# mpieva/mapping-iterative-assembler

Hardware: AMD Instinct MI355X
Metric: reads aligned/sec per iteration (16.5kb mito ref, 100bp reads) (higher is better)
Workload: dtype int32; 1 GPU; configs[1]: 1000000 synthetic 100 bp reads per GPU vs mt311 (16619 bp, circular), matrix flat; step = reiterate_assembly + pop_smp + cull + consensus; pass-1 coordinates = true positions; reads_per_gpu=1000000, total_reads=1000000, consensus_len=16619, bytes_per_read=182

## Files before the change

mapping-iterative-assembler_amd/csrc/mia_consensus_kernels.h:

```cpp
#pragma once
#include <hip/hip_runtime.h>
#include <stdint.h>

#include "mia_kernels.h"
#include "mia_layout.h"

namespace mia {

struct TallyBuf {
  int32_t* tally;
  int32_t Lp;
  int32_t* gaps;
  uint64_t* events;
  int32_t* n_events;
  int32_t cap_events;
  uint32_t* flags;
};

struct RecGeom {
  int start_w, end, split, ncols_f, ncols_b;
};
MIA_HD inline RecGeom rec_geom(int as, int ae, int L) {
  RecGeom g;
  g.start_w = as;
  g.end = ae > L ? ae - L : ae;
  g.split = as > g.end;
  g.ncols_f = g.split ? (L - as) : (g.end - as + 1);
  g.ncols_b = g.split ? g.end + 1 : 0;
  return g;
}

__global__ void k_scan_blocks(ReadSet rs, int32_t L, int64_t* partial) {
  __shared__ int32_t sh[256];
  const int64_t base = ((int64_t)blockIdx.x * 256 + threadIdx.x) * 16;
  int32_t s = 0;
  for (int k = 0; k < 16; k++) {
    int64_t i = base + k;
    if (i < rs.n && rs.sk[i]) s += rec_geom(rs.as[i], rs.ae[i], L).split ? 2 : 1;
  }
  sh[threadIdx.x] = s;
  __syncthreads();
  for (int o = 128; o > 0; o >>= 1) {
    if ((int)threadIdx.x < o) sh[threadIdx.x] += sh[threadIdx.x + o];
    __syncthreads();
  }
  if (threadIdx.x == 0) partial[blockIdx.x] = sh[0];
}
__global__ __launch_bounds__(256) void k_scan_partials(int64_t* partial, int nb, int64_t base, int64_t* total, const int32_t* abort_if = nullptr) {
  if (abort_if && *abort_if != 0) return;
  __shared__ int64_t s_run[256];
  const int t = threadIdx.x, per = (nb + 255) / 256, b0 = t * per, b1 = b0 + per < nb ? b0 + per : nb;
  int64_t mine = 0;
  for (int b = b0; b < b1; b++) mine += partial[b];
  const int lane = t & 63, w = t >> 6;
  int64_t inc = mine;
#pragma unroll
  for (int o = 1; o < 64; o <<= 1) { const int64_t u = (int64_t)__shfl_up((long long)inc, o); if (lane >= o) inc += u; }
  if (lane == 63) s_run[w] = inc;
// ... 782 lines not shown
    if (e < last) {
      const int32_t v = order[e];
      rd[q] = packed ? (v & 0xFFFFFF) : v;
      key[q] = packed ? (int)((uint32_t)v >> 24) : (int)okey[e];
      rank[q] = atomicAdd(&h[key[q]], 1);
    }
  }
  const int mine = pre[t];
  for (int o = 1; o < SORT2_KEYS; o <<= 1) {
    __syncthreads();
    const int v = t >= o ? pre[t - o] : 0;
    __syncthreads();
    pre[t] += v;
  }
  __syncthreads();
  pre[t] -= mine;
  base[t] = h[t] ? atomicAdd(&cursor2[(int64_t)b * SORT2_KEYS + t], h[t]) : 0;
  __syncthreads();
  const int ob = off[b];
#pragma unroll
  for (int q = 0; q < PER; q++)
    if (rd[q] >= 0) order2[ob + pre[key[q]] + base[key[q]] + rank[q]] = rd[q];
}

#ifdef MIA_HIP_ALT_PATHS
__device__ unsigned long long g_tally_kinds[8];
#define TALLY_KIND(k) do { if (dbg & 65536u) atomicAdd(&g_tally_kinds[k], 1ull); } while (0)
__device__ unsigned long long g_tally_clk[8];
#define TALLY_CLK(k) do { if ((dbg & 131072u) && threadIdx.x == 0) { const unsigned long long now_ = __builtin_amdgcn_s_memtime(); atomicAdd(&g_tally_clk[k], now_ - clk_); clk_ = now_; } } while (0)
#define TALLY_CLK_DECL unsigned long long clk_ = (dbg & 131072u) ? __builtin_amdgcn_s_memtime() : 0ull
#define TALLY_ABL(bit) ((dbg & (bit)) != 0u)
#else
#define TALLY_ABL(bit) false
#define TALLY_KIND(k) do { } while (0)
#define TALLY_CLK(k) do { } while (0)
#define TALLY_CLK_DECL do { } while (0)
#endif
__device__ __forceinline__ uint32_t wave_transpose32(uint32_t x, int lane) {
#pragma unroll
  for (int j = 16; j >= 1; j >>= 1) {
    const uint32_t m = j == 16 ? 0x0000FFFFu : (j == 8 ? 0x00FF00FFu : (j == 4 ? 0x0F0F0F0Fu : (j == 2 ? 0x33333333u : 0x55555555u)));
    const uint32_t y = (uint32_t)__shfl_xor((int)x, j);
    x = (lane & j) ? ((x & ~m) | ((y >> j) & m)) : ((x & m) | ((y << j) & ~m));
  }
  return x;
}

template <bool LINEAR, bool DEFER, bool RALL = false>
__global__ __launch_bounds__(256, 3) void k_tally_binned(ReadSet rs, RefInfo ref, const int32_t* pssm2, const uint8_t* drop_front,
                                                       const uint8_t* drop_back, TallyBuf tb, int32_t nb, const int32_t* off,
                                                       const int32_t* wgoff, const int32_t* order, const int32_t* rec_params,
                                                       const int32_t* rec_actf, int32_t* slabs, uint32_t dbg, const uint64_t* rplanes,
                                                       int32_t rplane_words, const int32_t* umax, const int32_t* wg_bucket, int32_t pk_bias, const int32_t* abort_if = nullptr,
                                                       int32_t chunk_reads = TALLY_CHUNK, int32_t* gen_list = nullptr, int32_t* n_gen = nullptr, int32_t split_flags = 0) {
  if (abort_if && *abort_if != 0) return;
  constexpr bool linear = LINEAR;
  const int split = split_flags & 1;
  const bool runs_on = !LINEAR && (split_flags & 2) != 0;
  __shared__ int32_t lds[(TALLY_WORDS - 1) * TALLY_WIN];
  __shared__ int32_t mid_cnt[LINEAR ? 1 : 5 * TALLY_WIN];
  __shared__ unsigned long long pk1[LINEAR ? 1 : TALLY_WIN], pk2[LINEAR ? 1 : TALLY_WIN];
  static_assert(TALLY_CHUNK <= 512, "packed end-base sums: 512 adds of at most 2047 stay below 2^20");
  __shared__ int32_t n_cnt[TALLY_WIN];
  __shared__ int32_t rec_stage[4][16];
  __shared__ int16_t pssm_lds[2 * PSSM_WORDS];
  __shared__ int32_t cov_diff[TALLY_WIN], span_diff[TALLY_WIN];
  __shared__ unsigned long long ev_buf[TALLY_EV_CAP];
  __shared__ int ev_cnt, ev_base;
  __shared__ unsigned long long run_tab[LINEAR ? 1 : (2 * PSSM_DEPTH + 1) * 4 * 2];
  if ((int)blockIdx.x >= wgoff[nb]) return;
  TALLY_CLK_DECL;
  const int4 wgi = reinterpret_cast<const int4*>(wg_bucket)[blockIdx.x];
  const int b = wgi.x >> split, first = wgi.y, last = wgi.z;
  const int wg_rc = split ? (wgi.x & 1) : 0;
  (void)wg_rc;
  const int win_base = b * TALLY_BUCKET;
  (void)off; (void)chunk_reads;
  int i_nx = first + (int)threadIdx.x < last ? order[first + (int)threadIdx.x] : -1;
  int i_nx2 = first + 256 + (int)threadIdx.x < last ? order[first + 256 + (int)threadIdx.x] : -1;
  for (int k = threadIdx.x; k < (TALLY_WORDS - 1) * TALLY_WIN; k += blockDim.x) lds[k] = 0;
  for (int k = threadIdx.x; k < ((LINEAR && DEFER) ? 25 : 2 * PSSM_WORDS); k += blockDim.x) pssm_lds[k] = (int16_t)pssm2[k];
  for (int k = threadIdx.x; k < TALLY_WIN; k += blockDim.x) { cov_diff[k] = 0; span_diff[k] = 0; n_cnt[k] = 0; }
  if (!LINEAR) for (int k = threadIdx.x; k < 5 * TALLY_WIN; k += blockDim.x) mid_cnt[k] = 0;
  if (!LINEAR) for (int k = threadIdx.x; k < TALLY_WIN; k += blockDim.x) { pk1[k] = 0; pk2[k] = 0; }
  if (threadIdx.x == 0) ev_cnt = 0;
  __syncthreads();
  if (!LINEAR && runs_on && pk_bias >= 0) {
    for (int k = threadIdx.x; k < (2 * PSSM_DEPTH + 1) * 4; k += blockDim.x) {
      const int16_t* row = pssm_lds + (wg_rc ? PSSM_WORDS : 0) + (k >> 2) * 25 + (k & 3);
      run_tab[2 * k] = (unsigned long long)(uint32_t)((int)row[0] + pk_bias) | ((unsigned long long)(uint32_t)((int)row[5] + pk_bias) << 20) |
                       ((unsigned long long)(uint32_t)((int)row[10] + pk_bias) << 40);
      run_tab[2 * k + 1] = (unsigned long long)(uint32_t)((int)row[15] + pk_bias) | (1ull << (20 + 10 * (k & 3)));
    }
    __syncthreads();
  }
  TALLY_CLK(0);
  const int lane = threadIdx.x & 63, wv = threadIdx.x >> 6;
  (void)wv;
  typedef __attribute__((address_space(3))) int32_t lds_i32;
  auto aadd = [](lds_i32* q, int v) { (void)__hip_atomic_fetch_add(q, v, __ATOMIC_RELAXED, __HIP_MEMORY_SCOPE_AGENT); };
  auto add_base = [&](int wc, int code, int d, bool is_rc, bool pack_ok = true) {
    lds_i32* t = (lds_i32*)lds + wc;
    if (LINEAR) { if (code < 4) aadd(&t[(T_A + code) * TALLY_WIN], 1); else aadd((lds_i32*)n_cnt + wc, 1); return; }
    if (d == PSSM_DEPTH) { aadd((lds_i32*)mid_cnt + (code < 4 ? code : 4) * TALLY_WIN + wc, is_rc ? 65536 : 1); return; }
    const int16_t* row = pssm_lds + (is_rc ? PSSM_WORDS : 0) + d * 25 + code;
    if (pk_bias >= 0 && code < 4 && pack_ok) {
      typedef __attribute__((address_space(3))) unsigned long long lds_u64;
      const unsigned long long v1 = (unsigned long long)(uint32_t)((int)row[0] + pk_bias) | ((unsigned long long)(uint32_t)((int)row[5] + pk_bias) << 20) |
                                    ((unsigned long long)(uint32_t)((int)row[10] + pk_bias) << 40);
      const unsigned long long v2 = (unsigned long long)(uint32_t)((int)row[15] + pk_bias) | (1ull << (20 + 10 * code));
      (void)__hip_atomic_fetch_add((lds_u64*)pk1 + wc, v1, __ATOMIC_RELAXED, __HIP_MEMORY_SCOPE_AGENT);
      (void)__hip_atomic_fetch_add((lds_u64*)pk2 + wc, v2, __ATOMIC_RELAXED, __HIP_MEMORY_SCOPE_AGENT);
      return;
    }
    if (code < 4) aadd(&t[(T_A + code) * TALLY_WIN], 1);
    aadd(&t[T_SA * TALLY_WIN], (int)row[0]);
    aadd(&t[T_SC * TALLY_WIN], (int)row[5]);
    aadd(&t[T_SG * TALLY_WIN], (int)row[10]);
    aadd(&t[T_ST * TALLY_WIN], (int)row[15]);
  };
  const int L = ref.L, Lp = tb.Lp;
  int warm = 0;
  constexpr int BS_W = 4;
  unsigned long long bs0[4 * BS_W], bs1[4 * BS_W];
  static_assert(!(LINEAR && RALL), "RALL is a mode of the position-specific tally");
  const bool bs_on = !RALL && (LINEAR || split != 0) && rplanes && umax && !(dbg & 4096u);
  const bool planes_all = RALL && split != 0 && rplanes && umax;
  auto bs_count = [&](unsigned long long l0, unsigned long long l1, unsigned long long h0, unsigned long long h1, int r_lo, int n_rows, int c) {
    const int rs_ = r_lo & 63;
    const bool rw = r_lo >= 64;
    auto down = [&](unsigned long long a0, unsigned long long a1, unsigned long long* o0, unsigned long long* o1) {
      const unsigned long long b0 = rw ? a1 : a0, b1 = rw ? 0ull : a1;
      *o0 = (b0 >> rs_) | ((b1 << 1) << (63 - rs_));
      *o1 = b1 >> rs_;
    };
    unsigned long long dl0, dl1, dh0, dh1;
    down(l0, l1, &dl0, &dl1); down(h0, h1, &dh0, &dh1);
    const unsigned long long v0 = n_rows >= 64 ? ~0ull : ((1ull << n_rows) - 1ull);
// ... 599 lines not shown
    const int item = (lane >> 2) & 15, bx_ = item / BS_W, wd = item % BS_W, c0 = (lane & 3) * 16;
#pragma unroll
    for (int j = 0; j < 16; j++) {
      int v = 0;
#pragma unroll
      for (int q = 0; q < 8; q++) v |= (int)((a8[q] >> (c0 + j)) & 1ull) << q;
      if (v) {
        if (LINEAR) aadd((lds_i32*)lds + (T_A + bx_) * TALLY_WIN + wd * 64 + c0 + j, v);
        else aadd((lds_i32*)mid_cnt + bx_ * TALLY_WIN + wd * 64 + c0 + j, wg_rc ? v << 16 : v);
      }
    }
  }
  if (warm == 0x7FFFFFF1) atomicOr(tb.flags, 4u);
  TALLY_CLK(2);
  __syncthreads();
  TALLY_CLK(3);
  const int ne = ev_cnt < TALLY_EV_CAP ? ev_cnt : TALLY_EV_CAP;
  int ev_base_reg = 0;
  if (threadIdx.x == 255 && ne > 0) ev_base_reg = atomicAdd(tb.n_events, ne);
  static_assert(TALLY_WIN == 64 * 6, "the difference arrays are scanned six entries per lane");
  if (wv < 2) {
    int32_t* d = wv == 0 ? cov_diff : span_diff;
    int32_t e[6], sum = 0;
#pragma unroll
    for (int q = 0; q < 6; q++) { e[q] = d[lane * 6 + q]; sum += e[q]; }
    int32_t inc = sum;
#pragma unroll
    for (int o = 1; o < 64; o <<= 1) { const int32_t u = __shfl_up(inc, o); if (lane >= o) inc += u; }
    int32_t run = inc - sum;
#pragma unroll
    for (int q = 0; q < 6; q++) { run += e[q]; d[lane * 6 + q] = run; }
  }
  __syncthreads();
  for (int k = threadIdx.x; k < TALLY_WIN; k += blockDim.x) { lds[T_COV * TALLY_WIN + k] += cov_diff[k]; lds[T_SPAN * TALLY_WIN + k] += span_diff[k]; }
  if (!LINEAR) {
    for (int k = threadIdx.x; k < TALLY_WIN; k += blockDim.x) {
      int sc[4] = {0, 0, 0, 0};
      for (int b5 = 0; b5 < 5; b5++) {
        const uint32_t w = (uint32_t)mid_cnt[b5 * TALLY_WIN + k];
        const int cf = (int)(w & 0xFFFFu), cr = (int)(w >> 16);
        if (b5 < 4) lds[(T_A + b5) * TALLY_WIN + k] += cf + cr;
        for (int x = 0; x < 4; x++)
          sc[x] += cf * (int)pssm_lds[PSSM_DEPTH * 25 + x * 5 + b5] + cr * (int)pssm_lds[PSSM_WORDS + PSSM_DEPTH * 25 + x * 5 + b5];
      }
      const unsigned long long p1 = pk1[k], p2 = pk2[k];
      int cnt = 0;
      for (int b5 = 0; b5 < 4; b5++) { const int c = (int)((p2 >> (20 + 10 * b5)) & 1023ull); lds[(T_A + b5) * TALLY_WIN + k] += c; cnt += c; }
      const int off = pk_bias > 0 ? pk_bias * cnt : 0;
      sc[0] += (int)(p1 & 0xFFFFFull) - off; sc[1] += (int)((p1 >> 20) & 0xFFFFFull) - off; sc[2] += (int)((p1 >> 40) & 0xFFFFFull) - off;
      sc[3] += (int)(p2 & 0xFFFFFull) - off;
      lds[T_SA * TALLY_WIN + k] += sc[0]; lds[T_SC * TALLY_WIN + k] += sc[1]; lds[T_SG * TALLY_WIN + k] += sc[2]; lds[T_ST * TALLY_WIN + k] += sc[3];
    }
  }
  if (linear) {
    for (int k = threadIdx.x; k < TALLY_WIN; k += blockDim.x) {
      int c[5];
      for (int b5 = 0; b5 < 4; b5++) c[b5] = lds[(T_A + b5) * TALLY_WIN + k];
      c[4] = n_cnt[k];
      const int rows[4] = {T_SA, T_SC, T_SG, T_ST};
      for (int x = 0; x < 4; x++) {
        int acc = 0;
        for (int b5 = 0; b5 < 5; b5++) acc += c[b5] * (int)pssm_lds[x * 5 + b5];
        lds[rows[x] * TALLY_WIN + k] += acc;
      }
    }
  }
  if (threadIdx.x == 255) ev_base = ev_base_reg;
  __syncthreads();
  TALLY_CLK(4);
  int32_t* slab = slabs + (int64_t)blockIdx.x * ((TALLY_WORDS - 1) * TALLY_WIN);
  if (!TALLY_ABL(1u << 20))
  for (int k = threadIdx.x; k < (TALLY_WORDS - 1) * TALLY_WIN; k += blockDim.x) slab[k] = lds[k];
  for (int k = threadIdx.x; k < ne; k += blockDim.x) {
    if (ev_base + k < tb.cap_events) tb.events[ev_base + k] = ev_buf[k]; else atomicOr(tb.flags, 1u);
  }
  TALLY_CLK(5);
#ifdef MIA_HIP_ALT_PATHS
  if ((dbg & 131072u) && threadIdx.x == 0) atomicAdd(&g_tally_clk[7], 1ull);
#endif
}

struct GenReads {
  ReadSet rs; RefInfo ref; const int32_t* pssm2; const uint8_t* drop_front; const uint8_t* drop_back; const int32_t* rec_params; const int32_t* rec_actf;
  const int32_t* list; const int32_t* n;
};
constexpr int TALLY_GEN_BLOCKS = 192;
constexpr int TALLY_REDUCE_SHARES = 4;
__global__ __launch_bounds__(256) void k_tally_reduce(TallyBuf tb, int32_t nb, const int32_t* wgoff, const int32_t* slabs, const int32_t* abort_if, GenReads gen, int32_t split = 0) {
  if (abort_if && *abort_if != 0) return;
  const int Lp = tb.Lp;
  const int gen_blocks = gen.list ? TALLY_GEN_BLOCKS : 0;
  if ((int)blockIdx.x < gen_blocks) {
    if (blockIdx.y != 0 || blockIdx.z != 0) return;
    const int lane = threadIdx.x & 63, wv = threadIdx.x >> 6, n = *gen.n;
    for (int k = (int)blockIdx.x * 4 + wv; k < n; k += TALLY_GEN_BLOCKS * 4)
      tally_one_read<false>(__builtin_amdgcn_readfirstlane(gen.list[k]), lane, gen.rs, gen.ref, gen.pssm2, gen.drop_front, gen.drop_back, tb, nullptr, 0, gen.rec_params,
                            gen.rec_actf, nullptr, nullptr, nullptr);
    return;
  }
  const int gc = ((int)blockIdx.x - gen_blocks) * blockDim.x + threadIdx.x, w = blockIdx.y;
  const int zs = blockIdx.z, zn = gridDim.z;
  if (gc >= Lp) return;
  int acc = 0;
  nb >>= split;
  const int bhi = min(gc / TALLY_BUCKET, nb - 1);
  for (int b = max(0, gc / TALLY_BUCKET - (TALLY_WIN / TALLY_BUCKET - 1)); b <= bhi; b++) {
    const int wc = gc - b * TALLY_BUCKET;
    if (wc < 0 || wc >= TALLY_WIN) continue;
    for (int wg = wgoff[b << split] + zs; wg < wgoff[(b + 1) << split]; wg += zn) acc += slabs[(int64_t)wg * ((TALLY_WORDS - 1) * TALLY_WIN) + w * TALLY_WIN + wc];
  }
  for (int b = max(0, (Lp + gc - TALLY_WIN) / TALLY_BUCKET); b < nb; b++) {
    const int wc = gc + Lp - b * TALLY_BUCKET;
    if (wc < 0 || wc >= TALLY_WIN || gc >= b * TALLY_BUCKET) continue;
    for (int wg = wgoff[b << split] + zs; wg < wgoff[(b + 1) << split]; wg += zn) acc += slabs[(int64_t)wg * ((TALLY_WORDS - 1) * TALLY_WIN) + w * TALLY_WIN + wc];
  }
  if (acc) (void)__hip_atomic_fetch_add(&tb.tally[w * Lp + gc], acc, __ATOMIC_RELAXED, __HIP_MEMORY_SCOPE_AGENT);
}

struct MaRecords {
  int64_t n;
  const int32_t* start;
  const uint8_t* revcom;
  const int64_t* col_off;
  const char* seq;
  const char* smp;
};
__device__ __forceinline__ int ma_code(char b) {
  return b == 'A' ? 0 : b == 'C' ? 1 : b == 'G' ? 2 : b == 'T' ? 3 : b == '-' ? 5 : 4;
}
__global__ __launch_bounds__(256) void k_ma_tally(MaRecords mr, const int32_t* pssm2, TallyBuf tb) {
  const int lane = threadIdx.x & 63;
  const int64_t r = (int64_t)blockIdx.x * 4 + (threadIdx.x >> 6);
  if (r >= mr.n) return;
  const int64_t o0 = mr.col_off[r];
  const int ncols = (int)(mr.col_off[r + 1] - o0), start = mr.start[r], Lp = tb.Lp;
  const int32_t* pm = pssm2 + (mr.revcom[r] ? PSSM_WORDS : 0);
  for (int p = lane; p < ncols; p += 64) {
    const int gc = start + p;
    if (gc < 0 || gc >= Lp) { atomicOr(tb.flags, 2u); continue; }
    const int code = ma_code(mr.seq[o0 + p]), d = (int)mr.smp[o0 + p] - 'A';
    int32_t* t = tb.tally + gc;
    atomicAdd(&t[T_COV * Lp], 1);
    if (code == 5) atomicAdd(&t[T_GAP * Lp], 1);
    else {
      if (d < 0 || d > 2 * PSSM_DEPTH) { atomicOr(tb.flags, 2u); continue; }
      if (code < 4) atomicAdd(&t[(T_A + code) * Lp], 1);
      const int32_t* row = pm + d * 25 + code;
      atomicAdd(&t[T_SA * Lp], row[0]);
      atomicAdd(&t[T_SC * Lp], row[5]);
      atomicAdd(&t[T_SG * Lp], row[10]);
      atomicAdd(&t[T_ST * Lp], row[15]);
    }
    if (p > 0) atomicAdd(&t[T_SPAN * Lp], 1);
  }
}
__global__ void k_ma_ins_events(MaRecords mr, int64_t n_ins, const int32_t* ins_record, const int32_t* ins_pos, const int64_t* ins_off,
                                const char* ins_bases, TallyBuf tb) {
  const int64_t e = (int64_t)blockIdx.x * blockDim.x + threadIdx.x;
  if (e >= n_ins) return;
  const int r = ins_record[e], p = ins_pos[e];
  const int64_t o0 = mr.col_off[r];
  const int ncols = (int)(mr.col_off[r + 1] - o0);
  if (p <= 0 || p >= ncols) return;
  const int gc = mr.start[r] + p, d = (int)mr.smp[o0 + p] - 'A';
  if (gc >= tb.Lp || d < 0 || d > 2 * PSSM_DEPTH) { atomicOr(tb.flags, 2u); return; }
  const int len = (int)(ins_off[e + 1] - ins_off[e]);
  for (int j = 0; j < len && j < 1024; j++) {
    const int code = ma_code(ins_bases[ins_off[e] + j]);
    const int slot = atomicAdd(tb.n_events, 1);
// ... 73 lines not shown
```

mapping-iterative-assembler_amd/csrc/mia_hip.hip:

```cpp
#include <hip/hip_runtime.h>
#include <atomic>
#include <hip/hip_ext.h>
#include <stdio.h>
#include <stdlib.h>
#include <string.h>

#include <algorithm>
#include <cmath>
#include <chrono>
#include <string>
#include <thread>
#include <vector>

#include "../../include/mia_hip.h"
#include "dev_buf.h"
#include "mia_comm.h"
#include "mia_consensus_kernels.h"
#include "mia_kernels.h"
#include "bandx_kernels.h"
#include "align_route.h"
#include "mia_pass1_kernels.h"
#include "mia_myers_kernels.h"
#include "mia_trim_kernels.h"
#include "mia_peak_kernels.h"
// ... 110 lines not shown
  DevBuf<BxCandRec> d_bx_cand2; int use_fine = 1;
  uint32_t* d_bx_ctr = nullptr;
  DevBuf<uint32_t> d_bx_slabs;
  int bx_values_wgs = 0, bx_trace_wgs = 0;
  DevBuf<uint32_t> d_bx_slabs_late; int bx_late_wgs = 0;
  DevBuf<uint32_t> d_bx_slabs_late2;
  DevBuf<int32_t> d_retry2;
  bool diag_scripts_missing = false;
  int64_t bx_seen = 0, bx_done[3] = {0, 0, 0};
  int64_t bx_launches = 0;
  uint32_t bx_last[BXC_COUNTERS] = {0};

  DevBuf<int64_t> d_slot, d_partial, d_total;
  DevBuf<uint8_t> d_slot_dropped, d_drop_f, d_drop_b; int64_t n_slots = 0;
  DevBuf<int64_t> d_back_slot;
  DevBuf<int64_t> d_front_slot0;
  DevBuf<int32_t> d_link_act;
  RecInfo ri{};
  DevBuf<int32_t> d_ri_flen, d_ri_blen, d_ri_actf, d_ri_trec;
  SlotInfo si{};
  DevBuf<int32_t> d_si_reclen, d_si_recact, d_si_mult; DevBuf<unsigned long long> d_si_writer;
  Links lk{};
  DevBuf<int64_t> d_lk_rec;
  int64_t* d_links_all = nullptr; int32_t n_links_all = 0;
  int32_t* d_n_links_all = nullptr; int64_t links_cap_all = 0; DevBuf<int32_t> d_n_links_gathered;
  DevBuf<int32_t> d_link_len;
  uint32_t* d_cull_flags = nullptr;
  DevBuf<uint32_t> d_cull_sync;
  DevBuf<unsigned long long> d_sums;
  int64_t read_base = 0;
  int64_t slot_base = 0;
  bool culled = false, links_applied = false;
  std::vector<DevBuf<int64_t>> owned_links;
  bool cull_scan = false, tail_scans = false;
  bool cull_with_records = true;
  int64_t pre_cull_records = 0, pre_cull_links = 0; bool pre_cull_valid = false;

  TallyBuf tb{}; DevBuf<int32_t> d_tb_tally, d_ins_off, d_ins_total; DevBuf<uint64_t> d_tb_events;
  DevBuf<int32_t> d_ins_tally; DevBuf<char> d_calls, d_ins_calls;
  int64_t ins_tally_cap = 0;
  int32_t n_events_host = 0; bool tallied = false;
  int64_t ins_total_host = 0;
  bool consensus_done = false;
  bool fake_event_overflow = false;
  bool no_linear_tally = false, sort2_unpacked = false;
  bool tally_linear = false;
  int tally_pk_bias = -1;
  int use_binned_tally = 1;
  DevBuf<int32_t> d_bucket, d_order;
  int bucket_clean_nb = -1;
  int buckets_queued = 0;
  bool no_side_buckets = false;
  DevBuf<int32_t> d_tally_slabs;
  DevBuf<int32_t> d_gen_list;
  bool tally_defer = true;
  bool tally_strand_split = true;
  bool tally_rall = true;
  bool tally_runs = true;
  DevBuf<int32_t> d_order2; DevBuf<uint8_t> d_okey; DevBuf<int32_t> d_sort2;

  bool in_iterate = false;
  const int32_t* abort_if = nullptr;
  bool spec_ok = false, spec_pending = false, spec_filtered = false, spec_bx = false, spec_plain = false;
  int64_t spec_redone = 0;
  bool no_spec = false;
  bool spec_force = false; DevBuf<int32_t> d_one;
  bool pend_encode = false; int32_t pend_L = 0, pend_wl = 0, pend_total = 0;
  bool zero_copy = true;
  const double* dev_cut = nullptr; DevBuf<double> d_cut_buf;
  DevBuf<char> d_ascii; const char* ascii_src = nullptr;
  DevBuf<char> d_cons;
  DevBuf<int32_t> d_cons_pos;
  unsigned char* h_pin2 = nullptr; size_t pin2_bytes = 0;
  int64_t iter_fallbacks = 0;

  double pass1_ms = 0; int64_t pass1_filtered = 0, pass1_anchored = 0;
  double myers_kernel_ms = 0; bool myers_no_lanes = false, myers_no_ond = false;
  int64_t trim_escapes = 0;
  bool ma_resident = false; int64_t ma_n = 0, ma_n_ins = 0; int32_t ma_L = 0;
  DevBuf<int32_t> d_ma_start, d_ma_gaps, d_ma_ipos, d_ma_rec_ins, d_ma_ins_list;
  DevBuf<int64_t> d_ma_coff, d_ma_ioff, d_ma_colmap, d_ma_rows;
  DevBuf<char> d_ma_seq, d_ma_ib, d_ma_text;
  DevBuf<unsigned long long> d_ma_ctl;
  int32_t ma_first = 0, ma_last = -1; int64_t ma_rows = 0, ma_width = 0; bool ma_region_done = false;
  bool ma_ace_gaps_ok = false, ma_ace_cols_ok = false, ma_ace_done = false; int64_t ma_ace_bytes = 0;
  DevBuf<int64_t> d_ace_g, d_ace_af, d_ace_len, d_ace_off; DevBuf<char> d_ace_body;
  bool ma_sam_gaps_ok = false, ma_sam_done = false; int64_t ma_sam_bytes = 0;
  DevBuf<char> d_sam_ref, d_sam_body; DevBuf<int64_t> d_sam_cum, d_sam_cig, d_sam_off; DevBuf<int32_t> d_sam_nm;
  DevBuf<unsigned long long> d_sam_ctl;
  DevBuf<uint8_t> d_ma_rev, d_prof_use; DevBuf<char> d_ma_smp, d_prof_ref; DevBuf<unsigned long long> d_prof_bins;
  bool ma_prof_done = false; int64_t ma_cols = 0; int64_t ma_prof_bins[MA_PROF_BINS] = {0};
  DevBuf<uint8_t> d_ends_seg; DevBuf<unsigned long long> d_ends_bins;
  bool ma_ends_done = false; int64_t ma_ends_bins[MA_ENDS_BINS] = {0};

  mia_hip_collectives coll{}; bool comm = false; int comm_ranks = 1, comm_rank = 0; std::string coll_name;
  DevBuf<unsigned long long> d_gather;
  std::vector<int64_t> h_gather;
  int64_t ev_pad = 0;
  DevBuf<int64_t> d_lstage, d_lmine, d_lall;
  DevBuf<int32_t> d_scores_all;
};

static void read_alt_switches(mia_hip_ctx* ctx) {
  auto on = [](const char* name) { const char* v = alt_env(name); return v && atoi(v) != 0; };
  if (on("MIA_HIP_NO_DIAG_FILTER")) { ctx->use_filter = 0; ctx->use_bx = 0; }
  if (on("MIA_HIP_NO_BAND_DP")) { ctx->use_banddp = 0; ctx->use_bx = 0; }
// ... 1606 lines not shown
  if (4 * (nb + 1) + 4 * grid > ctx->d_bucket.cap) {
    if (dev_alloc(ctx, ctx->d_bucket, (int64_t)(4 * (nb + 1) + 4 * grid) * 2)) return MIA_HIP_ERR_NOMEM;
    ctx->bucket_clean_nb = -1;
  }
  if (!ctx->d_order && dev_alloc(ctx, ctx->d_order, n)) return MIA_HIP_ERR_NOMEM;
  int32_t *d_cnt = ctx->d_bucket, *d_off = d_cnt + (nb + 1), *d_wgoff = d_off + (nb + 1), *d_cur = d_wgoff + (nb + 1), *d_wgb = d_cur + (nb + 1);
  if (ctx->bucket_clean_nb != nb) { HIPCHK(hipMemsetAsync(d_cnt, 0, (size_t)(nb + 1) * 4, on)); ctx->bucket_clean_nb = nb; }
  const int gb = (int)((n + 256 * BUCKET_PER - 1) / (256 * BUCKET_PER));
  hipLaunchKernelGGL(k_bucket_count, dim3(gb), dim3(256), (size_t)nb * 4, on, ctx->rs, nb, d_cnt, ctx->tb.tally, tally_words, ctx->abort_if, split);
  hipLaunchKernelGGL(k_bucket_scan, dim3(1), dim3(256), 0, on, d_cnt, nb, d_off, d_wgoff, d_cur, d_wgb, ctx->abort_if, chunk);
  const bool sigb = on != ctx->stream && (ctx->ext_events & 16u);
  if (!split) launch_k(k_bucket_fill, dim3(gb), dim3(256), (size_t)nb * 8, on, sigb ? ctx->ev_join : nullptr, ctx->rs, nb, d_off, d_cur, ctx->d_order, ctx->abort_if, split, (uint8_t*)nullptr, 0);
  else {
    const int64_t words2 = (int64_t)nb * SORT2_KEYS * 2;
    if (dev_ensure(ctx, ctx->d_sort2, words2)) return MIA_HIP_ERR_NOMEM;
    if (!ctx->d_order2 && dev_alloc(ctx, ctx->d_order2, n)) return MIA_HIP_ERR_NOMEM;
    if (!ctx->d_okey && dev_alloc(ctx, ctx->d_okey, n + 64)) return MIA_HIP_ERR_NOMEM;
    HIPCHK(hipMemsetAsync(ctx->d_sort2, 0, (size_t)words2 * 4, on));
    const int32_t packed = (n < (1 << 24) && !ctx->sort2_unpacked) ? 1 : 0;
    hipLaunchKernelGGL(k_bucket_fill, dim3(gb), dim3(256), (size_t)nb * 8, on, ctx->rs, nb, (const int32_t*)d_off, d_cur, ctx->d_order, ctx->abort_if, split, ctx->d_okey, packed);
    hipLaunchKernelGGL(k_sort2_count, dim3(grid), dim3(256), 0, on, nb, (const int32_t*)d_wgoff, (const int32_t*)d_wgb, (const int32_t*)ctx->d_order, (const uint8_t*)ctx->d_okey, packed,
                       ctx->d_sort2, ctx->abort_if);
    launch_k(k_sort2_fill, dim3(grid), dim3(256), 0, on, sigb ? ctx->ev_join : nullptr, nb, (const int32_t*)d_off, (const int32_t*)d_wgoff, (const int32_t*)d_wgb,
             (const int32_t*)ctx->d_order, (const uint8_t*)ctx->d_okey, packed, (const int32_t*)ctx->d_sort2, ctx->d_sort2 + (int64_t)nb * SORT2_KEYS, ctx->d_order2, ctx->abort_if);
  }
  HIPCHK(hipGetLastError());
  if (on != ctx->stream && !sigb) HIPCHK(hipEventRecord(ctx->ev_join, on));
  ctx->buckets_queued = on != ctx->stream ? 2 : 1;
  return MIA_HIP_OK;
}

static int tally_launch(mia_hip_ctx* ctx) {
  if (!ctx->aligned) { ctx->err = "realign first"; return MIA_HIP_ERR_STATE; }
  if (!ctx->culled) { ctx->err = "cull first (the dropped bits and record parameters are its output)"; return MIA_HIP_ERR_STATE; }
  HIPCHK(hipSetDevice(ctx->device));
  int rc = ensure_tally(ctx);
  if (rc) return rc;
  const int Lp = ctx->tb.Lp;
  const int64_t tally_words = (int64_t)(TALLY_WORDS + 1) * Lp + 256;
  if (!ctx->in_iterate) HIPCHK(hipMemsetAsync(ctx->tb.n_events, 0, 8, ctx->stream));
  const int64_t n = ctx->rs.n;
  const bool binned = tally_is_binned(ctx);
  if (!binned) HIPCHK(hipMemsetAsync(ctx->tb.tally, 0, (size_t)tally_words * 4, ctx->stream));
  if (n > 0) {
    RefInfo ref{ctx->d_ref, ctx->L, ctx->wrap};
    const int nb = tally_nb(ctx), split = tally_split(ctx);
    if (binned) {
      if (!ctx->buckets_queued) { if (int rcb = bucket_launch(ctx, ctx->stream)) return rcb; }
      if (ctx->buckets_queued == 2) HIPCHK(hipStreamWaitEvent(ctx->stream, ctx->ev_join, 0));
      ctx->buckets_queued = 0;
      const int chunk = tally_chunk(ctx);
      const int grid = (int)(n / chunk) + nb + 1;
      int32_t *d_cnt = ctx->d_bucket, *d_off = d_cnt + (nb + 1), *d_wgoff = d_off + (nb + 1), *d_cur = d_wgoff + (nb + 1), *d_wgb = d_cur + (nb + 1);
      const int64_t slab_words = (int64_t)grid * (TALLY_WORDS - 1) * TALLY_WIN;
      if (dev_ensure(ctx, ctx->d_tally_slabs, slab_words)) return MIA_HIP_ERR_NOMEM;
      const bool planes_ok = ctx->umax_valid && ctx->rs.roff == ctx->d_roff && ctx->d_rplanes && ctx->d_umax;
      const bool defer = ctx->tally_defer;
      if (defer && dev_ensure(ctx, ctx->d_gen_list, n)) return MIA_HIP_ERR_NOMEM;
      int32_t* n_gen = ctx->d_ctrl + CTRL_GENN;
      if (defer && !ctx->in_iterate) HIPCHK(hipMemsetAsync(n_gen, 0, 4, ctx->stream));
#define MIA_TALLY_ARGS(PL, RW, UM, BIAS)                                                                                                              \
  dim3(grid), dim3(256), 0, ctx->stream, ctx->rs, ref, ctx->d_pssm, ctx->d_drop_f, ctx->d_drop_b, ctx->tb, nb, d_off, d_wgoff, split ? ctx->d_order2 : ctx->d_order, ctx->ri.trec, \
      ctx->ri.actf, ctx->d_tally_slabs, ctx->dbg, PL, RW, UM, d_wgb, BIAS, ctx->abort_if, chunk, defer ? ctx->d_gen_list : (int32_t*)nullptr, n_gen, split | ((split && ctx->tally_runs) ? 2 : 0)
      const uint64_t* pl_arg = planes_ok ? ctx->d_rplanes : nullptr;
      const int32_t* um_arg = planes_ok ? ctx->d_umax : nullptr;
      int rct;
      if (ctx->tally_linear)
        rct = defer ? stage_launch(ctx, STG_TALLY, k_tally_binned<true, true>, MIA_TALLY_ARGS(pl_arg, ctx->rplane_words, um_arg, -1))
                    : stage_launch(ctx, STG_TALLY, k_tally_binned<true, false>, MIA_TALLY_ARGS(pl_arg, ctx->rplane_words, um_arg, -1));
      else if (split && tally_rall(ctx))
        rct = defer ? stage_launch(ctx, STG_TALLY, k_tally_binned<false, true, true>, MIA_TALLY_ARGS(pl_arg, ctx->rplane_words, um_arg, ctx->tally_pk_bias))
                    : stage_launch(ctx, STG_TALLY, k_tally_binned<false, false, true>, MIA_TALLY_ARGS(pl_arg, ctx->rplane_words, um_arg, ctx->tally_pk_bias));
      else
        rct = defer ? stage_launch(ctx, STG_TALLY, k_tally_binned<false, true>, MIA_TALLY_ARGS(split ? pl_arg : nullptr, ctx->rplane_words, split ? um_arg : nullptr, ctx->tally_pk_bias))
                    : stage_launch(ctx, STG_TALLY, k_tally_binned<false, false>, MIA_TALLY_ARGS(split ? pl_arg : nullptr, ctx->rplane_words, split ? um_arg : nullptr, ctx->tally_pk_bias));
#undef MIA_TALLY_ARGS
      if (rct) return MIA_HIP_ERR_NOMEM;
      GenReads gen{ctx->rs, ref, ctx->d_pssm, ctx->d_drop_f, ctx->d_drop_b, ctx->ri.trec, ctx->ri.actf, defer ? ctx->d_gen_list : nullptr, n_gen};
      hipLaunchKernelGGL(k_tally_reduce, dim3((Lp + 255) / 256 + (defer ? TALLY_GEN_BLOCKS : 0), TALLY_WORDS - 1, TALLY_REDUCE_SHARES), dim3(256), 0, ctx->stream, ctx->tb, nb, d_wgoff,
                         ctx->d_tally_slabs, ctx->abort_if, gen, split);
    } else {
      hipLaunchKernelGGL(k_tally, dim3((int)((n + 3) / 4)), dim3(256), 0, ctx->stream, ctx->rs, ref, ctx->d_pssm, ctx->d_drop_f,
                         ctx->d_drop_b, ctx->tb, ctx->ri.trec, ctx->ri.actf);
    }
    HIPCHK(hipGetLastError());
  }
  return MIA_HIP_OK;
}

static int tally_finish(mia_hip_ctx* ctx, uint32_t n_events, uint32_t flags, uint32_t cflags) {
  ctx->n_events_host = (int32_t)n_events;
  if (int rcf = check_cull_flags(ctx, cflags)) return rcf;
  if (flags & 1u) { ctx->err = "insert event list overflow"; return MIA_HIP_ERR_NOMEM; }
  if (ctx->n_events_host > ctx->tb.cap_events) ctx->n_events_host = ctx->tb.cap_events;
  ctx->tallied = true;
  ctx->consensus_done = false;
  return MIA_HIP_OK;
}

extern "C" int mia_hip_tally(mia_hip_ctx* ctx) {
  if (!ctx) return MIA_HIP_ERR_ARG;
  if (int rc = tally_launch(ctx)) return rc;
  uint32_t local3[3] = {0, 0, 0};
  uint32_t* h3 = ctx->h_pin ? reinterpret_cast<uint32_t*>(ctx->h_pin + (17 << 10)) : local3;
  HIPCHK(hipMemcpyAsync(&h3[0], ctx->tb.n_events, 4, hipMemcpyDeviceToHost, ctx->stream));
  HIPCHK(hipMemcpyAsync(&h3[1], ctx->tb.flags, 4, hipMemcpyDeviceToHost, ctx->stream));
  HIPCHK(hipMemcpyAsync(&h3[2], ctx->d_cull_flags, 4, hipMemcpyDeviceToHost, ctx->stream));
  HIPCHK(hipStreamSynchronize(ctx->stream));
  return tally_finish(ctx, h3[0], h3[1], h3[2]);
}

extern "C" int mia_hip_tally_buffers(mia_hip_ctx* ctx, int32_t** d_tally, int64_t* n_tally_words, int32_t** d_gaps,
                                     int64_t* n_gaps_words) {
  if (!ctx || !ctx->tallied) return MIA_HIP_ERR_STATE;
  if (d_tally) *d_tally = ctx->tb.tally;
  if (n_tally_words) *n_tally_words = (int64_t)TALLY_WORDS * ctx->tb.Lp;
  if (d_gaps) *d_gaps = ctx->tb.gaps;
  if (n_gaps_words) *n_gaps_words = ctx->tb.Lp;
  return MIA_HIP_OK;
}

extern "C" int mia_hip_ins_events(mia_hip_ctx* ctx, uint64_t** d_events, int64_t* n_events) {
  if (!ctx || !ctx->tallied) return MIA_HIP_ERR_STATE;
  if (d_events) *d_events = ctx->tb.events;
  if (n_events) *n_events = ctx->n_events_host;
  return MIA_HIP_OK;
}

extern "C" int mia_hip_set_ins_events(mia_hip_ctx* ctx, const uint64_t* d_events, int64_t n_events) {
  if (!ctx || !ctx->tallied || n_events < 0) return MIA_HIP_ERR_STATE;
  HIPCHK(hipSetDevice(ctx->device));
  if (n_events > ctx->tb.cap_events && ensure_events(ctx, n_events)) return MIA_HIP_ERR_NOMEM;
  if (n_events > 0 && d_events != ctx->tb.events)
// ... 118 lines not shown
```

Before: 1.434 billion reads/s.

## Pack linear tally slabs into 16-bit counts and reduce scores from summed counts

In the linear tally path, each workgroup now packs its eight per-column counts (A,C,G,T,N,gap,cov,span) into four 16-bit-pair words and writes only the used prefix of the window. The per-column score rows are no longer stored. A new packed reduce kernel sums the compact slabs per column, visiting only the workgroups whose windows overlap that column, and derives the PSSM scores from the summed counts, which is valid because the scores are linear in the counts. This cuts slab write and read traffic by nearly a factor of three and skips empty tails. If any count exceeds 16 bits, the workgroup falls back to direct global atomics, which costs extra code complexity.

```diff
diff --git a/mapping-iterative-assembler_amd/csrc/mia_consensus_kernels.h b/mapping-iterative-assembler_amd/csrc/mia_consensus_kernels.h
--- a/mapping-iterative-assembler_amd/csrc/mia_consensus_kernels.h
+++ b/mapping-iterative-assembler_amd/csrc/mia_consensus_kernels.h
@@ -4,6 +4,7 @@
 
 #include "mia_kernels.h"
 #include "mia_layout.h"
+#include "tally_slab.h"
 
 namespace mia {
 
@@ -892,7 +893,8 @@
                                                        const int32_t* wgoff, const int32_t* order, const int32_t* rec_params,
                                                        const int32_t* rec_actf, int32_t* slabs, uint32_t dbg, const uint64_t* rplanes,
                                                        int32_t rplane_words, const int32_t* umax, const int32_t* wg_bucket, int32_t pk_bias, const int32_t* abort_if = nullptr,
-                                                       int32_t chunk_reads = TALLY_CHUNK, int32_t* gen_list = nullptr, int32_t* n_gen = nullptr, int32_t split_flags = 0) {
+                                                       int32_t chunk_reads = TALLY_CHUNK, int32_t* gen_list = nullptr, int32_t* n_gen = nullptr, int32_t split_flags = 0,
+                                                       int32_t* slab_used = nullptr) {
   if (abort_if && *abort_if != 0) return;
   constexpr bool linear = LINEAR;
   const int split = split_flags & 1;
@@ -907,6 +909,7 @@
   __shared__ int32_t cov_diff[TALLY_WIN], span_diff[TALLY_WIN];
   __shared__ unsigned long long ev_buf[TALLY_EV_CAP];
   __shared__ int ev_cnt, ev_base;
+  __shared__ int pk_used, pk_bad;
   __shared__ unsigned long long run_tab[LINEAR ? 1 : (2 * PSSM_DEPTH + 1) * 4 * 2];
   if ((int)blockIdx.x >= wgoff[nb]) return;
   TALLY_CLK_DECL;
@@ -923,7 +926,7 @@
   for (int k = threadIdx.x; k < TALLY_WIN; k += blockDim.x) { cov_diff[k] = 0; span_diff[k] = 0; n_cnt[k] = 0; }
   if (!LINEAR) for (int k = threadIdx.x; k < 5 * TALLY_WIN; k += blockDim.x) mid_cnt[k] = 0;
   if (!LINEAR) for (int k = threadIdx.x; k < TALLY_WIN; k += blockDim.x) { pk1[k] = 0; pk2[k] = 0; }
-  if (threadIdx.x == 0) ev_cnt = 0;
+  if (threadIdx.x == 0) { ev_cnt = 0; pk_used = 0; pk_bad = 0; }
   __syncthreads();
   if (!LINEAR && runs_on && pk_bias >= 0) {
     for (int k = threadIdx.x; k < (2 * PSSM_DEPTH + 1) * 4; k += blockDim.x) {
@@ -1629,25 +1632,61 @@
       lds[T_SA * TALLY_WIN + k] += sc[0]; lds[T_SC * TALLY_WIN + k] += sc[1]; lds[T_SG * TALLY_WIN + k] += sc[2]; lds[T_ST * TALLY_WIN + k] += sc[3];
     }
   }
+  constexpr int PK_PER = (TALLY_WIN + 255) / 256;
+  uint4 pkw[PK_PER];
   if (linear) {
-    for (int k = threadIdx.x; k < TALLY_WIN; k += blockDim.x) {
-      int c[5];
-      for (int b5 = 0; b5 < 4; b5++) c[b5] = lds[(T_A + b5) * TALLY_WIN + k];
-      c[4] = n_cnt[k];
-      const int rows[4] = {T_SA, T_SC, T_SG, T_ST};
-      for (int x = 0; x < 4; x++) {
-        int acc = 0;
-        for (int b5 = 0; b5 < 5; b5++) acc += c[b5] * (int)pssm_lds[x * 5 + b5];
-        lds[rows[x] * TALLY_WIN + k] += acc;
-      }
-    }
+    int hi = 0;
+    bool bad = false;
+#pragma unroll
+    for (int q = 0; q < PK_PER; q++) {
+      const int k = (int)threadIdx.x + q * 256;
+      pkw[q] = make_uint4(0u, 0u, 0u, 0u);
+      if (k < TALLY_WIN) {
+        const int32_t c[TS_COUNTS] = {lds[T_A * TALLY_WIN + k], lds[T_C * TALLY_WIN + k], lds[T_G * TALLY_WIN + k], lds[T_T * TALLY_WIN + k],
+                                      n_cnt[k], lds[T_GAP * TALLY_WIN + k], lds[T_COV * TALLY_WIN + k], lds[T_SPAN * TALLY_WIN + k]};
+        uint32_t o[TS_WORDS];
+        if (!tally_slab_pack(c, o)) bad = true;
+        pkw[q] = make_uint4(o[0], o[1], o[2], o[3]);
+        if (o[0] | o[1] | o[2] | o[3]) hi = k + 1;
+      }
+    }
+    if (hi) atomicMax(&pk_used, hi);
+    if (bad) pk_bad = 1;
   }
   if (threadIdx.x == 255) ev_base = ev_base_reg;
   __syncthreads();
   TALLY_CLK(4);
-  int32_t* slab = slabs + (int64_t)blockIdx.x * ((TALLY_WORDS - 1) * TALLY_WIN);
-  if (!TALLY_ABL(1u << 20))
-  for (int k = threadIdx.x; k < (TALLY_WORDS - 1) * TALLY_WIN; k += blockDim.x) slab[k] = lds[k];
+  if (linear) {
+    uint4* slab = reinterpret_cast<uint4*>(slabs) + (int64_t)blockIdx.x * TALLY_WIN;
+    const bool overflow = pk_bad != 0;
+    const int used = (overflow || TALLY_ABL(1u << 20)) ? 0 : pk_used;
+    if (threadIdx.x == 0 && slab_used) slab_used[blockIdx.x] = used;
+#pragma unroll
+    for (int q = 0; q < PK_PER; q++) {
+      const int k = (int)threadIdx.x + q * 256;
+      if (k < used) slab[k] = pkw[q];
+    }
+    if (overflow) {
+      const int Lp = tb.Lp;
+      for (int k = threadIdx.x; k < TALLY_WIN; k += blockDim.x) {
+        int gc = win_base + k;
+        if (gc >= Lp) gc -= Lp;
+        if (gc < 0 || gc >= Lp) continue;
+        const int32_t c[5] = {lds[T_A * TALLY_WIN + k], lds[T_C * TALLY_WIN + k], lds[T_G * TALLY_WIN + k], lds[T_T * TALLY_WIN + k], n_cnt[k]};
+        int32_t s[4];
+        tally_scores_from_counts(c, pssm_lds, s);
+        const int32_t v[TALLY_WORDS - 1] = {c[0], c[1], c[2], c[3], lds[T_GAP * TALLY_WIN + k], lds[T_COV * TALLY_WIN + k], s[0], s[1], s[2], s[3],
+                                            lds[T_SPAN * TALLY_WIN + k]};
+        static_assert(T_A == 0 && T_GAP == 4 && T_COV == 5 && T_SA == 6 && T_SPAN == 10, "v[] above is in the tally's word order");
+        for (int w = 0; w < TALLY_WORDS - 1; w++)
+          if (v[w]) (void)__hip_atomic_fetch_add(&tb.tally[w * Lp + gc], v[w], __ATOMIC_RELAXED, __HIP_MEMORY_SCOPE_AGENT);
+      }
+    }
+  } else {
+    int32_t* slab = slabs + (int64_t)blockIdx.x * ((TALLY_WORDS - 1) * TALLY_WIN);
+    if (!TALLY_ABL(1u << 20))
+    for (int k = threadIdx.x; k < (TALLY_WORDS - 1) * TALLY_WIN; k += blockDim.x) slab[k] = lds[k];
+  }
   for (int k = threadIdx.x; k < ne; k += blockDim.x) {
     if (ev_base + k < tb.cap_events) tb.events[ev_base + k] = ev_buf[k]; else atomicOr(tb.flags, 1u);
   }
@@ -1692,6 +1731,71 @@
     for (int wg = wgoff[b << split] + zs; wg < wgoff[(b + 1) << split]; wg += zn) acc += slabs[(int64_t)wg * ((TALLY_WORDS - 1) * TALLY_WIN) + w * TALLY_WIN + wc];
   }
   if (acc) (void)__hip_atomic_fetch_add(&tb.tally[w * Lp + gc], acc, __ATOMIC_RELAXED, __HIP_MEMORY_SCOPE_AGENT);
+}
+
+constexpr int TALLY_PACKED_COLS = 32, TALLY_PACKED_SHARES = 256 / TALLY_PACKED_COLS;
+static_assert(TS_COUNTS <= TALLY_PACKED_SHARES, "the sums: one thread per (count, column)");
+__global__ __launch_bounds__(256) void k_tally_reduce_packed(TallyBuf tb, int32_t nb, const int32_t* wgoff, const int32_t* wg_bucket, const uint4* slabs,
+                                                               const int32_t* slab_used, const int32_t* abort_if, GenReads gen) {
+  if (abort_if && *abort_if != 0) return;
+  const int Lp = tb.Lp;
+  const int gen_blocks = gen.list ? TALLY_GEN_BLOCKS : 0;
+  if ((int)blockIdx.x < gen_blocks) {
+    const int lane = threadIdx.x & 63, wv = threadIdx.x >> 6, n = *gen.n;
+    for (int k = (int)blockIdx.x * 4 + wv; k < n; k += TALLY_GEN_BLOCKS * 4)
+      tally_one_read<false>(__builtin_amdgcn_readfirstlane(gen.list[k]), lane, gen.rs, gen.ref, gen.pssm2, gen.drop_front, gen.drop_back, tb, nullptr, 0, gen.rec_params,
+                            gen.rec_actf, nullptr, nullptr, nullptr);
+    return;
+  }
+  const int col = (int)threadIdx.x % TALLY_PACKED_COLS, zs = (int)threadIdx.x / TALLY_PACKED_COLS, zn = TALLY_PACKED_SHARES;
+  const int gc = ((int)blockIdx.x - gen_blocks) * TALLY_PACKED_COLS + col;
+  const bool live = gc < Lp;
+  int32_t acc[TS_COUNTS] = {0, 0, 0, 0, 0, 0, 0, 0};
+  if (live) {
+    auto take = [&](int wg) {
+      int wc = gc - wg_bucket[4 * wg] * TALLY_BUCKET;
+      if (wc < 0) wc += Lp;
+      uint4 v = make_uint4(0u, 0u, 0u, 0u);
+      if ((unsigned)wc < (unsigned)slab_used[wg]) v = slabs[(int64_t)wg * TALLY_WIN + wc];
+      return v;
+    };
+    auto add = [&](const uint4& v) { const uint32_t in[TS_WORDS] = {v.x, v.y, v.z, v.w}; tally_slab_unpack_add(in, acc); };
+    auto sum_range = [&](int w0, int w1) {
+      int wg = w0 + zs;
+      for (; wg + 3 * zn < w1; wg += 4 * zn) {
+        const uint4 v0 = take(wg), v1 = take(wg + zn), v2 = take(wg + 2 * zn), v3 = take(wg + 3 * zn);
+        add(v0); add(v1); add(v2); add(v3);
+      }
+      for (; wg < w1; wg += zn) add(take(wg));
+    };
+    const int gb = gc / TALLY_BUCKET;
+    const int d_lo = max(0, gb - (TALLY_WIN / TALLY_BUCKET - 1)), d_hi = min(gb, nb - 1);
+    const int c_lo = max(max(0, (Lp + gc - TALLY_WIN) / TALLY_BUCKET), gb + 1);
+    const int dw0 = wgoff[d_lo], dw1 = wgoff[d_hi + 1], cw0 = wgoff[min(c_lo, nb)], cw1 = wgoff[nb];
+    sum_range(dw0, dw1);
+    sum_range(cw0, cw1);
+  }
+  __shared__ int32_t part[TALLY_PACKED_SHARES][TALLY_PACKED_COLS][TS_COUNTS + 1], tot[TALLY_PACKED_COLS][TS_COUNTS + 1];
+  for (int j = 0; j < TS_COUNTS; j++) part[zs][col][j] = acc[j];
+  __syncthreads();
+  const int j = zs;
+  if (j < TS_COUNTS) {
+    int32_t t = 0;
+    for (int q = 0; q < TALLY_PACKED_SHARES; q++) t += part[q][col][j];
+    tot[col][j] = t;
+  }
+  __syncthreads();
+  if (!live || j >= TS_COUNTS) return;
+  auto out = [&](int w, int32_t v) { if (v) (void)__hip_atomic_fetch_add(&tb.tally[w * Lp + gc], v, __ATOMIC_RELAXED, __HIP_MEMORY_SCOPE_AGENT); };
+  if (j < 4) {
+    const int32_t c5[5] = {tot[col][TS_A], tot[col][TS_C], tot[col][TS_G], tot[col][TS_T], tot[col][TS_N]};
+    int32_t s[4];
+    tally_scores_from_counts(c5, gen.pssm2, s);
+    out(T_A + j, tot[col][j]);
+    out(T_SA + j, s[j]);
+  } else if (j == TS_GAP) out(T_GAP, tot[col][j]);
+  else if (j == TS_COV) out(T_COV, tot[col][j]);
+  else if (j == TS_SPAN) out(T_SPAN, tot[col][j]);
 }
 
 struct MaRecords {
diff --git a/mapping-iterative-assembler_amd/csrc/mia_hip.hip b/mapping-iterative-assembler_amd/csrc/mia_hip.hip
--- a/mapping-iterative-assembler_amd/csrc/mia_hip.hip
+++ b/mapping-iterative-assembler_amd/csrc/mia_hip.hip
@@ -186,6 +186,7 @@
   int buckets_queued = 0;
   bool no_side_buckets = false;
   DevBuf<int32_t> d_tally_slabs;
+  DevBuf<int32_t> d_tally_used;
   DevBuf<int32_t> d_gen_list;
   bool tally_defer = true;
   bool tally_strand_split = true;
@@ -1898,8 +1899,9 @@
       const int chunk = tally_chunk(ctx);
       const int grid = (int)(n / chunk) + nb + 1;
       int32_t *d_cnt = ctx->d_bucket, *d_off = d_cnt + (nb + 1), *d_wgoff = d_off + (nb + 1), *d_cur = d_wgoff + (nb + 1), *d_wgb = d_cur + (nb + 1);
-      const int64_t slab_words = (int64_t)grid * (TALLY_WORDS - 1) * TALLY_WIN;
+      const int64_t slab_words = (int64_t)grid * (ctx->tally_linear ? TS_WORDS : TALLY_WORDS - 1) * TALLY_WIN;
       if (dev_ensure(ctx, ctx->d_tally_slabs, slab_words)) return MIA_HIP_ERR_NOMEM;
+      if (ctx->tally_linear && dev_ensure(ctx, ctx->d_tally_used, grid)) return MIA_HIP_ERR_NOMEM;
       const bool planes_ok = ctx->umax_valid && ctx->rs.roff == ctx->d_roff && ctx->d_rplanes && ctx->d_umax;
       const bool defer = ctx->tally_defer;
       if (defer && dev_ensure(ctx, ctx->d_gen_list, n)) return MIA_HIP_ERR_NOMEM;
@@ -1907,7 +1909,8 @@
       if (defer && !ctx->in_iterate) HIPCHK(hipMemsetAsync(n_gen, 0, 4, ctx->stream));
 #define MIA_TALLY_ARGS(PL, RW, UM, BIAS)                                                                                                              \
   dim3(grid), dim3(256), 0, ctx->stream, ctx->rs, ref, ctx->d_pssm, ctx->d_drop_f, ctx->d_drop_b, ctx->tb, nb, d_off, d_wgoff, split ? ctx->d_order2 : ctx->d_order, ctx->ri.trec, \
-      ctx->ri.actf, ctx->d_tally_slabs, ctx->dbg, PL, RW, UM, d_wgb, BIAS, ctx->abort_if, chunk, defer ? ctx->d_gen_list : (int32_t*)nullptr, n_gen, split | ((split && ctx->tally_runs) ? 2 : 0)
+      ctx->ri.actf, ctx->d_tally_slabs, ctx->dbg, PL, RW, UM, d_wgb, BIAS, ctx->abort_if, chunk, defer ? ctx->d_gen_list : (int32_t*)nullptr, n_gen, split | ((split && ctx->tally_runs) ? 2 : 0), \
+      ctx->tally_linear ? (int32_t*)ctx->d_tally_used : (int32_t*)nullptr
       const uint64_t* pl_arg = planes_ok ? ctx->d_rplanes : nullptr;
       const int32_t* um_arg = planes_ok ? ctx->d_umax : nullptr;
       int rct;
@@ -1923,8 +1926,13 @@
 #undef MIA_TALLY_ARGS
       if (rct) return MIA_HIP_ERR_NOMEM;
       GenReads gen{ctx->rs, ref, ctx->d_pssm, ctx->d_drop_f, ctx->d_drop_b, ctx->ri.trec, ctx->ri.actf, defer ? ctx->d_gen_list : nullptr, n_gen};
-      hipLaunchKernelGGL(k_tally_reduce, dim3((Lp + 255) / 256 + (defer ? TALLY_GEN_BLOCKS : 0), TALLY_WORDS - 1, TALLY_REDUCE_SHARES), dim3(256), 0, ctx->stream, ctx->tb, nb, d_wgoff,
-                         ctx->d_tally_slabs, ctx->abort_if, gen, split);
+      if (ctx->tally_linear)
+        hipLaunchKernelGGL(k_tally_reduce_packed, dim3((Lp + TALLY_PACKED_COLS - 1) / TALLY_PACKED_COLS + (defer ? TALLY_GEN_BLOCKS : 0)), dim3(256), 0,
+                           ctx->stream, ctx->tb, nb, (const int32_t*)d_wgoff, (const int32_t*)d_wgb, reinterpret_cast<const uint4*>(ctx->d_tally_slabs.p),
+                           (const int32_t*)ctx->d_tally_used, ctx->abort_if, gen);
+      else
+        hipLaunchKernelGGL(k_tally_reduce, dim3((Lp + 255) / 256 + (defer ? TALLY_GEN_BLOCKS : 0), TALLY_WORDS - 1, TALLY_REDUCE_SHARES), dim3(256), 0, ctx->stream, ctx->tb, nb, d_wgoff,
+                           ctx->d_tally_slabs, ctx->abort_if, gen, split);
     } else {
       hipLaunchKernelGGL(k_tally, dim3((int)((n + 3) / 4)), dim3(256), 0, ctx->stream, ctx->rs, ref, ctx->d_pssm, ctx->d_drop_f,
                          ctx->d_drop_b, ctx->tb, ctx->ri.trec, ctx->ri.actf);
diff --git a/mapping-iterative-assembler_amd/csrc/tally_slab.h b/mapping-iterative-assembler_amd/csrc/tally_slab.h
--- /dev/null
+++ b/mapping-iterative-assembler_amd/csrc/tally_slab.h
@@ -0,0 +1,43 @@
+#pragma once
+#include <stdint.h>
+
+#ifndef MIA_HD
+#if defined(__HIPCC__)
+#define MIA_HD __host__ __device__
+#else
+#define MIA_HD
+#endif
+#endif
+
+namespace mia {
+
+enum { TS_A = 0, TS_C, TS_G, TS_T, TS_N, TS_GAP, TS_COV, TS_SPAN, TS_COUNTS };
+constexpr int TS_WORDS = TS_COUNTS / 2;
+
+MIA_HD inline bool tally_slab_pack(const int32_t c[TS_COUNTS], uint32_t out[TS_WORDS]) {
+  uint32_t all = 0;
+  for (int k = 0; k < TS_WORDS; k++) {
+    const uint32_t lo = (uint32_t)c[2 * k], hi = (uint32_t)c[2 * k + 1];
+    all |= lo | hi;
+    out[k] = (lo & 0xFFFFu) | (hi << 16);
+  }
+  return (all >> 16) == 0;
+}
+
+MIA_HD inline void tally_slab_unpack_add(const uint32_t in[TS_WORDS], int32_t acc[TS_COUNTS]) {
+  for (int k = 0; k < TS_WORDS; k++) {
+    acc[2 * k] += (int32_t)(in[k] & 0xFFFFu);
+    acc[2 * k + 1] += (int32_t)(in[k] >> 16);
+  }
+}
+
+template <class T>
+MIA_HD inline void tally_scores_from_counts(const int32_t c[5], const T* sm, int32_t s[4]) {
+  for (int x = 0; x < 4; x++) {
+    int32_t acc = 0;
+    for (int b = 0; b < 5; b++) acc += c[b] * (int32_t)sm[x * 5 + b];
+    s[x] = acc;
+  }
+}
+
+}
```

New measurement: 1.466 billion reads/s, median of 6. 2.2% higher.
